# OSU-Nowlab/MPI4DL

Hardware: NVIDIA H100
Metric: images/sec (device-timed, max over ranks) AmoebaNet-D 8192^2 hot path (spatial-stage conv/pool fwd+bwd) (higher is better)
Workload: dtype bf16

## Files before the change

### mpi4dl_b200/build.py

```python
import os
import subprocess
import sys

HERE = os.path.dirname(os.path.abspath(__file__))
CSRC = os.path.join(HERE, "csrc")
LIB = os.path.join(HERE, "libspconv.so")
SOURCES = ["api.cu", "conv_direct.cu", "pool.cu", "halo.cu", "gemm_tc.cu", "conv_tap.cu", "wgrad_tap.cu", "bnrelu.cu",
           "halo_grad.cu", "gemm_tf32.cu", "conv_tap_tf32.cu", "conv_tap_s2_tf32.cu"]
NVCC_FLAGS = [
    "-O3", "-std=c++17", "-gencode", "arch=compute_90a,code=sm_90a", "-lineinfo",
    "-Xcompiler", "-fPIC", "--expt-relaxed-constexpr",
]


def _stale(target, deps):
    if not os.path.exists(target):
        return True
    t = os.path.getmtime(target)
    return any(os.path.getmtime(d) > t for d in deps)


def build_lib(force=False, verbose=False):
    nvcc = os.environ.get("NVCC", "/usr/local/cuda/bin/nvcc")
    hdrs = [os.path.join(CSRC, f) for f in os.listdir(CSRC) if f.endswith((".cuh", ".h"))]
    hdrs.append(os.path.join(HERE, "..", "include", "spconv.h"))
    objs = []
    procs = []
    for s in SOURCES:
        src = os.path.join(CSRC, s)
        obj = os.path.join(CSRC, s.replace(".cu", ".o"))
        objs.append(obj)
        if force or _stale(obj, [src] + hdrs):
            cmd = [nvcc] + NVCC_FLAGS + (["-Xptxas", "-v"] if verbose else []) + ["-c", src, "-o", obj]
            procs.append((s, subprocess.Popen(cmd, stdout=subprocess.PIPE, stderr=subprocess.STDOUT, text=True)))
    for s, p in procs:
        out, _ = p.communicate()
        if p.returncode != 0:
            sys.stderr.write(out)
            raise RuntimeError("nvcc failed on %s" % s)
        if verbose:
            sys.stderr.write(out)
    if force or procs or _stale(LIB, objs):
        cmd = [nvcc, "-shared", "-o", LIB] + objs + ["-gencode", "arch=compute_90a,code=sm_90a"]
        subprocess.check_call(cmd)
    return LIB


if __name__ == "__main__":
    print(build_lib(force="--force" in sys.argv, verbose="-v" in sys.argv))
```

### mpi4dl_b200/csrc/gemm_tc.cu

```cuda
#include <stdlib.h>

#include "common.cuh"
#include "tc_common.cuh"

namespace spc {

using namespace tc;

bool tap_v2_supported(int M, int Cin, int R, int S, int H, int W, int N, int stride);
int run_conv_tap_v2(const __nv_bfloat16* wp, int Mpad, int Cpad, const __nv_bfloat16* x, const __nv_bfloat16* bias,
                    __nv_bfloat16* y, int M, int Cin, int R, int S, int ph, int H, int W, int N, cudaStream_t st);

bool wgrad_tap_supported(int K, int C, int R, int S, int H, int W, int stride);
int run_wgrad_tap(const __nv_bfloat16* x, const __nv_bfloat16* dy, float* dw, int K, int C, int N, int H, int W, int R, int S,
                  cudaStream_t st);

namespace {

constexpr int TC_THREADS = 384;
constexpr int BK = 64;
constexpr int A_BLK_BYTES = 128 * BK * 2;
constexpr int B_BLK_BYTES = BK * 64 * 2;

typedef CUresult (*EncodeTiledFn)(CUtensorMap*, CUtensorMapDataType, cuuint32_t, void*, const cuuint64_t*,
                                  const cuuint64_t*, const cuuint32_t*, const cuuint32_t*, CUtensorMapInterleave,
                                  CUtensorMapSwizzle, CUtensorMapL2promotion, CUtensorMapFloatOOBfill);
EncodeTiledFn get_encode() {
  static EncodeTiledFn fn = nullptr;
  if (!fn) {
    void* p = nullptr;
    cudaDriverEntryPointQueryResult q;
    if (cudaGetDriverEntryPoint("cuTensorMapEncodeTiled", &p, cudaEnableDefault, &q) == cudaSuccess &&
        q == cudaDriverEntryPointSuccess)
      fn = reinterpret_cast<EncodeTiledFn>(p);
  }
  return fn;
}

int make_tmap_sw(CUtensorMap* m, const void* base, int rank, const uint64_t* dims, const uint64_t* strides_bytes,
                 const uint32_t* box, CUtensorMapSwizzle swz) {
  EncodeTiledFn enc = get_encode();
  if (!enc) {
    set_error("cuTensorMapEncodeTiled entry point not available");
    return SPC_ECUDA;
  }
  static thread_local bool ctx_bound = false;
  if (!ctx_bound) {
    if (cudaFree(nullptr) != cudaSuccess) {
      set_error("wgmma conv: no CUDA context on this thread");
      return SPC_ECUDA;
    }
    ctx_bound = true;
  }
  cuuint64_t gd[5], gs[5];
  cuuint32_t bx[5], es[5];
  for (int i = 0; i < rank; ++i) {
    gd[i] = dims[i];
    bx[i] = box[i];
    es[i] = 1;
    if (i > 0) gs[i - 1] = strides_bytes[i];
  }
  CUresult r = enc(m, CU_TENSOR_MAP_DATA_TYPE_BFLOAT16, (cuuint32_t)rank, const_cast<void*>(base), gd, gs, bx, es,
                   CU_TENSOR_MAP_INTERLEAVE_NONE, swz, CU_TENSOR_MAP_L2_PROMOTION_L2_256B,
                   CU_TENSOR_MAP_FLOAT_OOB_FILL_NONE);
  if (r != CUDA_SUCCESS) {
    set_error("cuTensorMapEncodeTiled failed (%d) rank=%d dims=[%llu,%llu,%llu] strides=[%llu,%llu]", (int)r, rank,
              (unsigned long long)dims[0], (unsigned long long)(rank > 1 ? dims[1] : 0),
              (unsigned long long)(rank > 2 ? dims[2] : 0), (unsigned long long)(rank > 1 ? strides_bytes[1] : 0),
              (unsigned long long)(rank > 2 ? strides_bytes[2] : 0));
    return SPC_ECUDA;
  }
  return SPC_OK;
}

int make_tmap(CUtensorMap* m, const void* base, int rank, const uint64_t* dims, const uint64_t* strides_bytes,
              const uint32_t* box) {
  return make_tmap_sw(m, base, rank, dims, strides_bytes, box, CU_TENSOR_MAP_SWIZZLE_128B);
}

__global__ void repack_weights_kernel(const __nv_bfloat16* __restrict__ w, __nv_bfloat16* __restrict__ wp, int M,
                                      int Cc, int Mpad, int Cpad, int taps, long long sm, long long sc, int flip) {
  const int total = taps * Mpad * Cpad;
  for (int i = blockIdx.x * blockDim.x + threadIdx.x; i < total; i += gridDim.x * blockDim.x) {
    const int c = i % Cpad;
    const int m = (i / Cpad) % Mpad;
    const int tap = i / (Cpad * Mpad);
    __nv_bfloat16 v = __float2bfloat16(0.f);
    if (m < M && c < Cc) v = w[(size_t)m * sm + (size_t)c * sc + (flip ? taps - 1 - tap : tap)];
    wp[i] = v;
  }
}

constexpr int BN = 128;
constexpr int OUT_BUF_BYTES = 128 * 128 * 2;
constexpr int MAX_STAGES = 8;

struct PwParams {
  int M;
// ... 187 lines not shown
struct EnvKnob { const char* name; const char* val; };
EnvKnob g_env_tab[32];
int g_env_n = 0;
inline const char* env_get(const char* name) {
  for (int i = 0; i < g_env_n; ++i)
    if (g_env_tab[i].name == name) return g_env_tab[i].val;
  const char* v = getenv(name);
  if (g_env_n < 32) { g_env_tab[g_env_n].name = name; g_env_tab[g_env_n].val = v; ++g_env_n; }
  return v;
}
inline int env_int(const char* name, int dflt) {
  const char* e = env_get(name);
  const int v = e ? atoi(e) : 0;
  return v > 0 ? v : dflt;
}
inline int sm_count() {
  static int sms = 0;
  if (!sms) {
    int dev = 0;
    cudaGetDevice(&dev);
    if (cudaDeviceGetAttribute(&sms, cudaDevAttrMultiProcessorCount, dev) != cudaSuccess || sms <= 0) sms = 132;
  }
  return sms;
}

constexpr int SMEM_LIMIT = 222 * 1024;
constexpr int SMEM_AUX = 1024  + 512 ;

template <int MB>
int launch_pw(const CUtensorMap& tw, const CUtensorMap& tx, const CUtensorMap& tx4, const CUtensorMap& ty, PwParams p,
              cudaStream_t st) {
  const int kchunks = (p.Cin + BK - 1) / BK;
  const int budget = SMEM_LIMIT - SMEM_AUX;
  const int wres_bytes = p.taps * kchunks * MB * A_BLK_BYTES;
  const int sms = sm_count();
  const int grid = p.num_tiles < sms ? p.num_tiles : sms;
  if (p.num_tiles < 16 * sms) p.tgroup = 1;
  p.wres = (wres_bytes <= 128 * 1024 && p.num_mg == 1) ? 1 : 0;
  const int stage_bytes = (p.wres ? 0 : MB * A_BLK_BYTES) + (BN / 64) * B_BLK_BYTES;
  const int rem = budget - (p.wres ? wres_bytes : 0);
  p.out_bufs = 2;
  p.stages = (rem - 2 * OUT_BUF_BYTES) / stage_bytes;
  if (p.stages < 3) { p.out_bufs = 1; p.stages = (rem - OUT_BUF_BYTES) / stage_bytes; }
  if (p.stages > MAX_STAGES) p.stages = MAX_STAGES;
  SPC_REQUIRE(p.stages >= 2, "wgmma conv: shared memory budget too small (MB=%d kchunks=%d)", MB, kchunks);
  const int smem = (p.wres ? wres_bytes : 0) + p.stages * stage_bytes + p.out_bufs * OUT_BUF_BYTES + SMEM_AUX;
  auto kern = pw_gemm_kernel<MB>;
  static bool attr_set = false;
  if (!attr_set) {
    SPC_CHECK_CUDA(cudaFuncSetAttribute(kern, cudaFuncAttributeMaxDynamicSharedMemorySize, SMEM_LIMIT));
    attr_set = true;
  }
  kern<<<grid, TC_THREADS, smem, st>>>(tw, tx, tx4, ty, p);
  count_launch();
  SPC_CHECK_CUDA(cudaGetLastError());
  return SPC_OK;
}

int make_act_tmap(CUtensorMap* m, const void* base, int P, int Cc, int N, int box_rows) {
  const uint64_t dims[3] = {(uint64_t)P, (uint64_t)Cc, (uint64_t)N};
  const uint64_t strides[3] = {0, (uint64_t)P * 2, (uint64_t)P * Cc * 2};
  const uint32_t box[3] = {64, (uint32_t)box_rows, 1};
  return make_tmap(m, base, 3, dims, strides, box);
}

int make_act_tmap5(CUtensorMap* m, const void* base, int P, int Cc, int N, int groups, int blocks) {
  const uint64_t dims[5] = {64, 8, (uint64_t)P / 64, (uint64_t)Cc / 8, (uint64_t)N};
  const uint64_t strides[5] = {0, (uint64_t)P * 2, 128, (uint64_t)P * 16, (uint64_t)P * Cc * 2};
  const uint32_t box[5] = {64, 8, (uint32_t)blocks, (uint32_t)groups, 1};
  return make_tmap(m, base, 5, dims, strides, box);
}

int launch_shift_copies(const void* x, void* xs, size_t planes, int H, int W, int S, int pw, int cs, cudaStream_t st);

struct TcConv {
  const __nv_bfloat16* w;
  long long sm, sc;
  int flip;
  int M, Cin;
  int R, S, ph, pw;
  int H, W, N;
  int stride;
  const __nv_bfloat16* prepacked;
};

int run_conv_tc(const TcConv& c, const __nv_bfloat16* x, const __nv_bfloat16* bias, __nv_bfloat16* y, void* ws,
                size_t ws_bytes, cudaStream_t st) {
  const int taps = c.R * c.S;
  const int cs = c.stride;
  const int Ho = c.H / cs, Wo = c.W / cs;
  const int Pin = c.H * c.W, P = Ho * Wo;
  const int Mpad = round_up(c.M, 128), Cpad = round_up(c.Cin, BK);
  const bool v2 = taps > 1 && !env_get("SPC_TAP_V1") && tap_v2_supported(c.M, c.Cin, c.R, c.S, c.H, c.W, c.N, cs);
  const bool copies = (c.S > 1 || cs > 1) && taps > 1 && !v2;
  const uintptr_t ws0 = reinterpret_cast<uintptr_t>(ws);
  const uintptr_t wp_addr = (ws0 + 1023) & ~(uintptr_t)1023;
  const size_t wp_bytes = c.prepacked ? 0 : (size_t)taps * Mpad * Cpad * 2;
  const uintptr_t xs_addr = (wp_addr + wp_bytes + 1023) & ~(uintptr_t)1023;
  const size_t xs_bytes = copies ? (size_t)c.S * c.N * c.Cin * c.H * Wo * 2 : 0;
  const size_t need = (xs_addr - ws0) + xs_bytes;
  SPC_REQUIRE((ws && ws_bytes >= need) || need <= 1024, "wgmma conv: workspace too small (%zu < %zu)", ws_bytes, need);
  const __nv_bfloat16* wp = c.prepacked;
  if (!c.prepacked) {
    __nv_bfloat16* wpm = reinterpret_cast<__nv_bfloat16*>(wp_addr);
    const int total = taps * Mpad * Cpad;
    int blocks = (total + 255) / 256;
    if (blocks > 1184) blocks = 1184;
    repack_weights_kernel<<<blocks, 256, 0, st>>>(c.w, wpm, c.M, c.Cin, Mpad, Cpad, taps, c.sm, c.sc, c.flip);
    count_launch();
    SPC_CHECK_CUDA(cudaGetLastError());
    wp = wpm;
  }
  if (v2)
    return run_conv_tap_v2(wp, Mpad, Cpad, x, bias, y, c.M, c.Cin, c.R, c.S, c.ph, c.H, c.W, c.N, st);
  const __nv_bfloat16* xsrc = x;
  if (copies) {
    void* xs = reinterpret_cast<void*>(xs_addr);
    int rc0 = launch_shift_copies(x, xs, (size_t)c.N * c.Cin, c.H, c.W, c.S, c.pw, cs, st);
    if (rc0) return rc0;
    xsrc = reinterpret_cast<const __nv_bfloat16*>(xs);
  }
  CUtensorMap tw, tx, tx4, ty;
  const char* box5_env = env_get("SPC_PW_BOX5");
  const int box5 = box5_env ? atoi(box5_env) : ((size_t)P * 2 >= ((size_t)4 << 20) ? 3 : 0);
  const int x5 = (taps == 1 && cs == 1 && (box5 & 1) && P % 64 == 0 && c.Cin % 8 == 0) ? 1 : 0;
  const int y5 = (taps == 1 && (box5 & 2) && P % 64 == 0 && c.M % 8 == 0) ? 1 : 0;
  {
    const uint64_t dims[2] = {(uint64_t)Cpad, (uint64_t)taps * Mpad};
    const uint64_t strides[2] = {0, (uint64_t)Cpad * 2};
    const uint32_t box[2] = {BK, 128};
    int rc = make_tmap(&tw, wp, 2, dims, strides, box);
    if (rc) return rc;
  }
  int rc;
  if (taps > 1) {
    const uint64_t dims[4] = {(uint64_t)Wo, (uint64_t)c.H, (uint64_t)c.Cin, (uint64_t)c.N * (copies ? c.S : 1)};
    const uint64_t strides[4] = {0, (uint64_t)Wo * 2, (uint64_t)c.H * Wo * 2, (uint64_t)c.H * Wo * c.Cin * 2};
    const uint32_t box[4] = {64, 1, BK, 1};
    rc = make_tmap(&tx4, xsrc, 4, dims, strides, box);
    if (rc) return rc;
    tx = tx4;
  } else {
    rc = x5 ? make_act_tmap5(&tx, x, Pin, c.Cin, c.N, BK / 8, BN / 64) : make_act_tmap(&tx, x, Pin, c.Cin, c.N, BK);
    if (rc) return rc;
    tx4 = tx;
  }
  rc = y5 ? make_act_tmap5(&ty, y, P, c.M, c.N, 16, 2) : make_act_tmap(&ty, y, P, c.M, c.N, 128);
  if (rc) return rc;
  PwParams p{};
  p.x5 = x5; p.y5 = y5;
  p.bias = bias; p.M = c.M; p.Cin = c.Cin; p.P = P; p.N = c.N;
  p.taps = taps; p.S = c.S; p.ph = c.ph; p.pw = c.pw; p.W = Wo; p.Mpad = Mpad;
  p.shiftN = copies ? c.N : 0;
  p.rowmul = cs;
  {
    const char* e = env_get("SPC_TILE_GROUP");
    p.tgroup = e ? atoi(e) : 1;
    if (p.tgroup < 1) p.tgroup = 1;
  }
  const int MBtot = Mpad / 128;
  const int mb = MBtot >= 2 ? 2 : 1;
  p.num_mg = (MBtot + mb - 1) / mb;
  p.tiles_per_image = (P + BN - 1) / BN;
  p.num_tiles = p.tiles_per_image * c.N * p.num_mg;
  return mb == 2 ? launch_pw<2>(tw, tx, tx4, ty, p, st) : launch_pw<1>(tw, tx, tx4, ty, p, st);
}

int run_pw(const __nv_bfloat16* w, int ld, int transpose, int M, int Cin, const __nv_bfloat16* x,
           const __nv_bfloat16* bias, __nv_bfloat16* y, int N, int P, void* ws, size_t ws_bytes, cudaStream_t st) {
  TcConv c{};
  c.w = w;
  c.sm = transpose ? 1 : ld; c.sc = transpose ? ld : 1; c.flip = 0;
  c.M = M; c.Cin = Cin; c.R = 1; c.S = 1; c.ph = 0; c.pw = 0; c.H = 1; c.W = P; c.N = N; c.stride = 1;
  return run_conv_tc(c, x, bias, y, ws, ws_bytes, st);
}

constexpr int WG_ACC = 256;

struct WgParams {
  float* dw;
  int K, C, P, N;
  int nblk;
  int n_blocks;
  int MG;
  int mgroups;
  int splits;
  int chunks_total;
  int chunks_per_image;
  int stages;
  int taps, S, ph;
  int TG, passes;
  int W, shiftN;
  int rowmul;
  int mrows;
  int split_major;
  int pb;
  int dy5, x5;
};

template <int NBLK, int NA>
__global__ void __launch_bounds__(TC_THREADS, 1)
pw_wgrad_kernel(const __grid_constant__ CUtensorMap tmap_dy, const __grid_constant__ CUtensorMap tmap_x,
                const __grid_constant__ CUtensorMap tmap_x4, const WgParams p) {
  static_assert(NA * NBLK <= WG_ACC, "accumulator registers");
  extern __shared__ uint8_t smem_raw[];
  uint8_t* smem = reinterpret_cast<uint8_t*>((reinterpret_cast<uintptr_t>(smem_raw) + 1023) & ~(uintptr_t)1023);
  const int MG = p.MG;
  const int b_bytes = NBLK * 128;
  const int b_slot = (b_bytes + 1023) & ~1023;
  const int stage_bytes = p.pb * (MG * A_BLK_BYTES + p.TG * b_slot);
  uint64_t* full = reinterpret_cast<uint64_t*>(smem + p.stages * stage_bytes);
  uint64_t* empty = full + MAX_STAGES;
  const int warp = threadIdx.x >> 5, lane = threadIdx.x & 31;

  if (threadIdx.x == 0) {
    for (int i = 0; i < p.stages; ++i) { mbar_init(&full[i], 1); mbar_init(&empty[i], 2); }
    fence_barrier_init();
  }
  __syncthreads();
  const int ngroups = p.mgroups * p.n_blocks * p.passes;
  const int num_items = ngroups * p.splits;
  const int per_split = (p.chunks_total + p.splits - 1) / p.splits;

#define WG_DECODE(it)                                                        \
  const int sp = p.split_major ? (it) / ngroups : (it) % p.splits;           \
  const int g_ = p.split_major ? (it) % ngroups : (it) / p.splits;           \
  const int pass = g_ % p.passes;                                            \
  const int nb = (g_ / p.passes) % p.n_blocks;                               \
  const int mgp = g_ / (p.passes * p.n_blocks);                              \
  const int tap0 = pass * p.TG;                                              \
  const int ntap = min(p.TG, p.taps - tap0);                                 \
  const int c_begin = sp * per_split, c_end = min(p.chunks_total, c_begin + per_split);

  if (warp == 0) {
    if (lane == 0) {
      tma_prefetch_desc(&tmap_dy);
      tma_prefetch_desc(&tmap_x);
      int s = 0, ph = 0;
      for (int it = blockIdx.x; it < num_items; it += gridDim.x) {
        WG_DECODE(it)
        for (int ch = c_begin; ch < c_end; ++ch) {
          const int n = ch / p.chunks_per_image, p0 = (ch % p.chunks_per_image) * (64 * p.pb);
          mbar_wait(&empty[s], ph ^ 1);
          uint8_t* st = smem + s * stage_bytes;
          mbar_arrive_expect_tx(&full[s], p.pb * (MG * p.mrows * 128 + ntap * b_bytes));
          if (p.pb == 2) {
            for (int i = 0; i < MG; ++i) {
              uint8_t* da = st + i * (2 * A_BLK_BYTES);
              const int r0 = (mgp * MG + i) * p.mrows;
              if (p.dy5) {
                tma_load_5d(da, &tmap_dy, &full[s], 0, 0, p0 >> 6, r0 >> 3, n);
              } else {
                tma_load_3d(da, &tmap_dy, &full[s], p0, r0, n);
// ... 549 lines not shown
    uintptr_t a = align1k(reinterpret_cast<uintptr_t>(ws));
    __nv_bfloat16* wq = reinterpret_cast<__nv_bfloat16*>(a);
    a = align1k(a + (size_t)4 * Mpad * Kpad * 2);
    __nv_bfloat16* tmp = reinterpret_cast<__nv_bfloat16*>(a);
    a = align1k(a + (size_t)4 * d->N * d->C * Ho * Wo * 2);
    {
      const int total = 4 * Mpad * Kpad;
      int blocks = (total + 255) / 256;
      if (blocks > 1184) blocks = 1184;
      repack_dgrad_s2_kernel<<<blocks, 256, 0, st>>>(reinterpret_cast<const __nv_bfloat16*>(w), wq, d->K, d->C, Mpad, Kpad);
      count_launch();
      SPC_CHECK_CUDA(cudaGetLastError());
    }
    TcConv c{};
    c.prepacked = wq;
    c.M = Mq; c.Cin = d->K; c.R = 2; c.S = 2; c.ph = 0; c.pw = 0; c.H = Ho; c.W = Wo; c.N = d->N; c.stride = 1;
    int rc = run_conv_tc(c, reinterpret_cast<const __nv_bfloat16*>(dy), nullptr, tmp, reinterpret_cast<void*>(a),
                         ws_bytes - (a - reinterpret_cast<uintptr_t>(ws)), st);
    if (rc) return rc;
    const size_t total = (size_t)d->N * d->C * 2 * Ho * (Wo / 8);
    size_t blocks = (total + 255) / 256;
    if (blocks > 132 * 32) blocks = 132 * 32;
    interleave_s2_kernel<<<(int)blocks, 256, 0, st>>>(tmp, reinterpret_cast<__nv_bfloat16*>(dx), d->N, d->C, Ho, Wo);
    count_launch();
    SPC_CHECK_CUDA(cudaGetLastError());
    return SPC_OK;
  }
  if (d->R * d->S > 1) {
    TcConv c{};
    c.w = reinterpret_cast<const __nv_bfloat16*>(w);
    c.sm = (long long)d->R * d->S; c.sc = (long long)d->C * d->R * d->S; c.flip = 1;
    c.M = d->C; c.Cin = d->K; c.R = d->R; c.S = d->S; c.ph = d->R - 1 - d->pad_h; c.pw = d->S - 1 - d->pad_w;
    c.H = d->H; c.W = d->W; c.N = d->N; c.stride = 1;
    return run_conv_tc(c, reinterpret_cast<const __nv_bfloat16*>(dy), nullptr, reinterpret_cast<__nv_bfloat16*>(dx), ws,
                       ws_bytes, st);
  }
  if (is_s2(d)) {
    void* gs = reinterpret_cast<void*>(align1k(reinterpret_cast<uintptr_t>(ws) + wbytes(d, 1)));
    int rc = run_pw(reinterpret_cast<const __nv_bfloat16*>(w), d->C, 1, d->C, d->K,
                    reinterpret_cast<const __nv_bfloat16*>(dy), nullptr, reinterpret_cast<__nv_bfloat16*>(gs), d->N,
                    (d->H / 2) * (d->W / 2), ws, wbytes(d, 1), st);
    if (rc) return rc;
    return launch_resample(true, gs, dx, (size_t)d->N * d->C, d->H, d->W, st);
  }
  return run_pw(reinterpret_cast<const __nv_bfloat16*>(w), d->C, 1, d->C, d->K,
                reinterpret_cast<const __nv_bfloat16*>(dy), nullptr, reinterpret_cast<__nv_bfloat16*>(dx), d->N,
                d->H * d->W, ws, ws_bytes, st);
}

int tc_conv_wgrad(const spc_conv_desc* d, const void* x, const void* dy, float* dw, int accumulate, void* ws,
                  size_t ws_bytes, cudaStream_t st) {
  (void)accumulate;
  const __nv_bfloat16* xb = reinterpret_cast<const __nv_bfloat16*>(x);
  const __nv_bfloat16* dyb = reinterpret_cast<const __nv_bfloat16*>(dy);
  if (d->R * d->S > 1) {
    const int cs = d->stride_h;
    if (!env_get("SPC_TAP_V1") && wgrad_tap_supported(d->K, d->C, d->R, d->S, d->H, d->W, cs))
      return run_wgrad_tap(xb, dyb, dw, d->K, d->C, d->N, d->H, d->W, d->R, d->S, st);
    const bool copies = d->S > 1 || cs > 1;
    if (copies) {
      SPC_REQUIRE(ws && ws_bytes >= tc_workspace_bytes(d, 2), "wgmma wgrad: workspace too small");
      void* xs = reinterpret_cast<void*>(align1k(reinterpret_cast<uintptr_t>(ws)));
      int rc = launch_shift_copies(x, xs, (size_t)d->N * d->C, d->H, d->W, d->S, d->pad_w, cs, st);
      if (rc) return rc;
      xb = reinterpret_cast<const __nv_bfloat16*>(xs);
    }
    return run_wgrad(xb, dyb, dw, d->K, d->C, d->N, d->H / cs, d->W / cs, d->H, d->R, d->S, d->pad_h, cs, copies, st);
  }
  if (is_s2(d)) {
    SPC_REQUIRE(ws && ws_bytes >= tc_workspace_bytes(d, 2), "wgmma wgrad: workspace too small");
    void* xs = reinterpret_cast<void*>(align1k(reinterpret_cast<uintptr_t>(ws)));
    int rc = launch_resample(false, x, xs, (size_t)d->N * d->C, d->H, d->W, st);
    if (rc) return rc;
    return run_wgrad(reinterpret_cast<const __nv_bfloat16*>(xs), dyb, dw, d->K, d->C, d->N, 1, (d->H / 2) * (d->W / 2), 1,
                     1, 1, 0, 1, false, st);
  }
  return run_wgrad(xb, dyb, dw, d->K, d->C, d->N, 1, d->H * d->W, 1, 1, 1, 0, 1, false, st);
}

size_t tc_pw_workspace_bytes(int M, int Cin) { return (size_t)round_up(M, 128) * round_up(Cin, BK) * 2 + 4096; }
int tc_pw_fwd(const void* w, int ld, int M, int Cin, const void* x, const void* bias, void* y, int P, void* ws, size_t ws_bytes,
              cudaStream_t st) {
  return run_pw(reinterpret_cast<const __nv_bfloat16*>(w), ld, 0, M, Cin, reinterpret_cast<const __nv_bfloat16*>(x),
                reinterpret_cast<const __nv_bfloat16*>(bias), reinterpret_cast<__nv_bfloat16*>(y), 1, P, ws, ws_bytes, st);
}
int tc_pw_wgrad(const void* x, const void* dy, float* dw, int K, int C, int P, cudaStream_t st) {
  return run_wgrad(reinterpret_cast<const __nv_bfloat16*>(x), reinterpret_cast<const __nv_bfloat16*>(dy), dw, K, C, 1, 1, P, 1, 1, 1,
                   0, 1, false, st);
}

int make_tmap_ex(CUtensorMap* m, const void* base, int rank, const uint64_t* dims, const uint64_t* strides_bytes,
                 const uint32_t* box, int swizzle128) {
  return make_tmap_sw(m, base, rank, dims, strides_bytes, box,
                      swizzle128 ? CU_TENSOR_MAP_SWIZZLE_128B : CU_TENSOR_MAP_SWIZZLE_NONE);
}
int tc_sm_count() { return sm_count(); }

}

extern "C" void spc_reload_env(void) { spc::g_env_n = 0; }
```

### mpi4dl_b200/csrc/wgmma.cuh

```cuda
#pragma once
#include <stdint.h>

namespace spc {
namespace tc {

template <int N, int TB> struct Wgmma;

template <int TB> struct Wgmma<16, TB> {
  static __device__ __forceinline__ void mma(float (&d)[8], uint64_t a, uint64_t b, uint32_t accumulate) {
    asm volatile(
        "{\n\t.reg .pred p;\n\t"
        "setp.ne.b32 p, %10, 0;\n\t"
        "wgmma.mma_async.sync.aligned.m64n16k16.f32.bf16.bf16 {%0, %1, %2, %3, %4, %5, %6, %7}, %8, %9, p, 1, 1, 0, %11;\n\t}"
        : "+f"(d[0]), "+f"(d[1]), "+f"(d[2]), "+f"(d[3]), "+f"(d[4]), "+f"(d[5]), "+f"(d[6]), "+f"(d[7])
        : "l"(a), "l"(b), "r"(accumulate), "n"(TB));
  }
};

template <int TB> struct Wgmma<32, TB> {
  static __device__ __forceinline__ void mma(float (&d)[16], uint64_t a, uint64_t b, uint32_t accumulate) {
    asm volatile(
        "{\n\t.reg .pred p;\n\t"
        "setp.ne.b32 p, %18, 0;\n\t"
        "wgmma.mma_async.sync.aligned.m64n32k16.f32.bf16.bf16 {%0, %1, %2, %3, %4, %5, %6, %7, %8, %9, %10, %11, %12, %13, %14, %15}, %16, %17, p, 1, 1, 0, %19;\n\t}"
        : "+f"(d[0]), "+f"(d[1]), "+f"(d[2]), "+f"(d[3]), "+f"(d[4]), "+f"(d[5]), "+f"(d[6]), "+f"(d[7]), "+f"(d[8]), "+f"(d[9]), "+f"(d[10]), "+f"(d[11]), "+f"(d[12]), "+f"(d[13]), "+f"(d[14]), "+f"(d[15])
        : "l"(a), "l"(b), "r"(accumulate), "n"(TB));
  }
};

template <int TB> struct Wgmma<48, TB> {
  static __device__ __forceinline__ void mma(float (&d)[24], uint64_t a, uint64_t b, uint32_t accumulate) {
    asm volatile(
        "{\n\t.reg .pred p;\n\t"
        "setp.ne.b32 p, %26, 0;\n\t"
        "wgmma.mma_async.sync.aligned.m64n48k16.f32.bf16.bf16 {%0, %1, %2, %3, %4, %5, %6, %7, %8, %9, %10, %11, %12, %13, %14, %15, %16, %17, %18, %19, %20, %21, %22, %23}, %24, %25, p, 1, 1, 0, %27;\n\t}"
        : "+f"(d[0]), "+f"(d[1]), "+f"(d[2]), "+f"(d[3]), "+f"(d[4]), "+f"(d[5]), "+f"(d[6]), "+f"(d[7]), "+f"(d[8]), "+f"(d[9]), "+f"(d[10]), "+f"(d[11]), "+f"(d[12]), "+f"(d[13]), "+f"(d[14]), "+f"(d[15]), "+f"(d[16]), "+f"(d[17]), "+f"(d[18]), "+f"(d[19]), "+f"(d[20]), "+f"(d[21]), "+f"(d[22]), "+f"(d[23])
        : "l"(a), "l"(b), "r"(accumulate), "n"(TB));
  }
};

template <int TB> struct Wgmma<64, TB> {
  static __device__ __forceinline__ void mma(float (&d)[32], uint64_t a, uint64_t b, uint32_t accumulate) {
    asm volatile(
        "{\n\t.reg .pred p;\n\t"
        "setp.ne.b32 p, %34, 0;\n\t"
        "wgmma.mma_async.sync.aligned.m64n64k16.f32.bf16.bf16 {%0, %1, %2, %3, %4, %5, %6, %7, %8, %9, %10, %11, %12, %13, %14, %15, %16, %17, %18, %19, %20, %21, %22, %23, %24, %25, %26, %27, %28, %29, %30, %31}, %32, %33, p, 1, 1, 0, %35;\n\t}"
        : "+f"(d[0]), "+f"(d[1]), "+f"(d[2]), "+f"(d[3]), "+f"(d[4]), "+f"(d[5]), "+f"(d[6]), "+f"(d[7]), "+f"(d[8]), "+f"(d[9]), "+f"(d[10]), "+f"(d[11]), "+f"(d[12]), "+f"(d[13]), "+f"(d[14]), "+f"(d[15]), "+f"(d[16]), "+f"(d[17]), "+f"(d[18]), "+f"(d[19]), "+f"(d[20]), "+f"(d[21]), "+f"(d[22]), "+f"(d[23]), "+f"(d[24]), "+f"(d[25]), "+f"(d[26]), "+f"(d[27]), "+f"(d[28]), "+f"(d[29]), "+f"(d[30]), "+f"(d[31])
        : "l"(a), "l"(b), "r"(accumulate), "n"(TB));
  }
};

template <int TB> struct Wgmma<80, TB> {
  static __device__ __forceinline__ void mma(float (&d)[40], uint64_t a, uint64_t b, uint32_t accumulate) {
    asm volatile(
        "{\n\t.reg .pred p;\n\t"
        "setp.ne.b32 p, %42, 0;\n\t"
        "wgmma.mma_async.sync.aligned.m64n80k16.f32.bf16.bf16 {%0, %1, %2, %3, %4, %5, %6, %7, %8, %9, %10, %11, %12, %13, %14, %15, %16, %17, %18, %19, %20, %21, %22, %23, %24, %25, %26, %27, %28, %29, %30, %31, %32, %33, %34, %35, %36, %37, %38, %39}, %40, %41, p, 1, 1, 0, %43;\n\t}"
        : "+f"(d[0]), "+f"(d[1]), "+f"(d[2]), "+f"(d[3]), "+f"(d[4]), "+f"(d[5]), "+f"(d[6]), "+f"(d[7]), "+f"(d[8]), "+f"(d[9]), "+f"(d[10]), "+f"(d[11]), "+f"(d[12]), "+f"(d[13]), "+f"(d[14]), "+f"(d[15]), "+f"(d[16]), "+f"(d[17]), "+f"(d[18]), "+f"(d[19]), "+f"(d[20]), "+f"(d[21]), "+f"(d[22]), "+f"(d[23]), "+f"(d[24]), "+f"(d[25]), "+f"(d[26]), "+f"(d[27]), "+f"(d[28]), "+f"(d[29]), "+f"(d[30]), "+f"(d[31]), "+f"(d[32]), "+f"(d[33]), "+f"(d[34]), "+f"(d[35]), "+f"(d[36]), "+f"(d[37]), "+f"(d[38]), "+f"(d[39])
        : "l"(a), "l"(b), "r"(accumulate), "n"(TB));
  }
};

template <int TB> struct Wgmma<96, TB> {
  static __device__ __forceinline__ void mma(float (&d)[48], uint64_t a, uint64_t b, uint32_t accumulate) {
    asm volatile(
        "{\n\t.reg .pred p;\n\t"
        "setp.ne.b32 p, %50, 0;\n\t"
        "wgmma.mma_async.sync.aligned.m64n96k16.f32.bf16.bf16 {%0, %1, %2, %3, %4, %5, %6, %7, %8, %9, %10, %11, %12, %13, %14, %15, %16, %17, %18, %19, %20, %21, %22, %23, %24, %25, %26, %27, %28, %29, %30, %31, %32, %33, %34, %35, %36, %37, %38, %39, %40, %41, %42, %43, %44, %45, %46, %47}, %48, %49, p, 1, 1, 0, %51;\n\t}"
        : "+f"(d[0]), "+f"(d[1]), "+f"(d[2]), "+f"(d[3]), "+f"(d[4]), "+f"(d[5]), "+f"(d[6]), "+f"(d[7]), "+f"(d[8]), "+f"(d[9]), "+f"(d[10]), "+f"(d[11]), "+f"(d[12]), "+f"(d[13]), "+f"(d[14]), "+f"(d[15]), "+f"(d[16]), "+f"(d[17]), "+f"(d[18]), "+f"(d[19]), "+f"(d[20]), "+f"(d[21]), "+f"(d[22]), "+f"(d[23]), "+f"(d[24]), "+f"(d[25]), "+f"(d[26]), "+f"(d[27]), "+f"(d[28]), "+f"(d[29]), "+f"(d[30]), "+f"(d[31]), "+f"(d[32]), "+f"(d[33]), "+f"(d[34]), "+f"(d[35]), "+f"(d[36]), "+f"(d[37]), "+f"(d[38]), "+f"(d[39]), "+f"(d[40]), "+f"(d[41]), "+f"(d[42]), "+f"(d[43]), "+f"(d[44]), "+f"(d[45]), "+f"(d[46]), "+f"(d[47])
        : "l"(a), "l"(b), "r"(accumulate), "n"(TB));
  }
};

template <int TB> struct Wgmma<112, TB> {
  static __device__ __forceinline__ void mma(float (&d)[56], uint64_t a, uint64_t b, uint32_t accumulate) {
    asm volatile(
        "{\n\t.reg .pred p;\n\t"
        "setp.ne.b32 p, %58, 0;\n\t"
        "wgmma.mma_async.sync.aligned.m64n112k16.f32.bf16.bf16 {%0, %1, %2, %3, %4, %5, %6, %7, %8, %9, %10, %11, %12, %13, %14, %15, %16, %17, %18, %19, %20, %21, %22, %23, %24, %25, %26, %27, %28, %29, %30, %31, %32, %33, %34, %35, %36, %37, %38, %39, %40, %41, %42, %43, %44, %45, %46, %47, %48, %49, %50, %51, %52, %53, %54, %55}, %56, %57, p, 1, 1, 0, %59;\n\t}"
        : "+f"(d[0]), "+f"(d[1]), "+f"(d[2]), "+f"(d[3]), "+f"(d[4]), "+f"(d[5]), "+f"(d[6]), "+f"(d[7]), "+f"(d[8]), "+f"(d[9]), "+f"(d[10]), "+f"(d[11]), "+f"(d[12]), "+f"(d[13]), "+f"(d[14]), "+f"(d[15]), "+f"(d[16]), "+f"(d[17]), "+f"(d[18]), "+f"(d[19]), "+f"(d[20]), "+f"(d[21]), "+f"(d[22]), "+f"(d[23]), "+f"(d[24]), "+f"(d[25]), "+f"(d[26]), "+f"(d[27]), "+f"(d[28]), "+f"(d[29]), "+f"(d[30]), "+f"(d[31]), "+f"(d[32]), "+f"(d[33]), "+f"(d[34]), "+f"(d[35]), "+f"(d[36]), "+f"(d[37]), "+f"(d[38]), "+f"(d[39]), "+f"(d[40]), "+f"(d[41]), "+f"(d[42]), "+f"(d[43]), "+f"(d[44]), "+f"(d[45]), "+f"(d[46]), "+f"(d[47]), "+f"(d[48]), "+f"(d[49]), "+f"(d[50]), "+f"(d[51]), "+f"(d[52]), "+f"(d[53]), "+f"(d[54]), "+f"(d[55])
        : "l"(a), "l"(b), "r"(accumulate), "n"(TB));
  }
};

template <int TB> struct Wgmma<128, TB> {
  static __device__ __forceinline__ void mma(float (&d)[64], uint64_t a, uint64_t b, uint32_t accumulate) {
    asm volatile(
        "{\n\t.reg .pred p;\n\t"
        "setp.ne.b32 p, %66, 0;\n\t"
        "wgmma.mma_async.sync.aligned.m64n128k16.f32.bf16.bf16 {%0, %1, %2, %3, %4, %5, %6, %7, %8, %9, %10, %11, %12, %13, %14, %15, %16, %17, %18, %19, %20, %21, %22, %23, %24, %25, %26, %27, %28, %29, %30, %31, %32, %33, %34, %35, %36, %37, %38, %39, %40, %41, %42, %43, %44, %45, %46, %47, %48, %49, %50, %51, %52, %53, %54, %55, %56, %57, %58, %59, %60, %61, %62, %63}, %64, %65, p, 1, 1, 0, %67;\n\t}"
        : "+f"(d[0]), "+f"(d[1]), "+f"(d[2]), "+f"(d[3]), "+f"(d[4]), "+f"(d[5]), "+f"(d[6]), "+f"(d[7]), "+f"(d[8]), "+f"(d[9]), "+f"(d[10]), "+f"(d[11]), "+f"(d[12]), "+f"(d[13]), "+f"(d[14]), "+f"(d[15]), "+f"(d[16]), "+f"(d[17]), "+f"(d[18]), "+f"(d[19]), "+f"(d[20]), "+f"(d[21]), "+f"(d[22]), "+f"(d[23]), "+f"(d[24]), "+f"(d[25]), "+f"(d[26]), "+f"(d[27]), "+f"(d[28]), "+f"(d[29]), "+f"(d[30]), "+f"(d[31]), "+f"(d[32]), "+f"(d[33]), "+f"(d[34]), "+f"(d[35]), "+f"(d[36]), "+f"(d[37]), "+f"(d[38]), "+f"(d[39]), "+f"(d[40]), "+f"(d[41]), "+f"(d[42]), "+f"(d[43]), "+f"(d[44]), "+f"(d[45]), "+f"(d[46]), "+f"(d[47]), "+f"(d[48]), "+f"(d[49]), "+f"(d[50]), "+f"(d[51]), "+f"(d[52]), "+f"(d[53]), "+f"(d[54]), "+f"(d[55]), "+f"(d[56]), "+f"(d[57]), "+f"(d[58]), "+f"(d[59]), "+f"(d[60]), "+f"(d[61]), "+f"(d[62]), "+f"(d[63])
        : "l"(a), "l"(b), "r"(accumulate), "n"(TB));
  }
};

}
}
```

Baseline: 3.227.

## Add pixel-major wgmma pointwise conv kernel with channel-sized N tiles

Adds a new warp-specialized wgmma GEMM for 1x1 convolutions where pixels form the M dimension (128 per tile) and output channels the N dimension, tiled at 56/104/208. It is used when the channel count pads poorly to 128-row tiles and there are enough tiles to fill the GPU. The intent is to cut wasted MMA work and padding for odd channel counts such as 52 or 208, and to keep weights resident in shared memory when they fit. The kernel uses transposed-A wgmma, stmatrix transpose for the epilogue, and TMA stores. It adds another code path and a layout, and it can run more slowly on shapes where the heuristic chooses poorly.

```diff
diff --git a/mpi4dl_b200/build.py b/mpi4dl_b200/build.py
--- a/mpi4dl_b200/build.py
+++ b/mpi4dl_b200/build.py
@@ -6,7 +6,8 @@
 CSRC = os.path.join(HERE, "csrc")
 LIB = os.path.join(HERE, "libspconv.so")
 SOURCES = ["api.cu", "conv_direct.cu", "pool.cu", "halo.cu", "gemm_tc.cu", "conv_tap.cu", "wgrad_tap.cu", "bnrelu.cu",
-           "halo_grad.cu", "gemm_tf32.cu", "conv_tap_tf32.cu", "conv_tap_s2_tf32.cu"]
+           "halo_grad.cu", "gemm_tf32.cu", "conv_tap_tf32.cu", "conv_tap_s2_tf32.cu",
+           "gemm_px.cu"]
 NVCC_FLAGS = [
     "-O3", "-std=c++17", "-gencode", "arch=compute_90a,code=sm_90a", "-lineinfo",
     "-Xcompiler", "-fPIC", "--expt-relaxed-constexpr",
diff --git a/mpi4dl_b200/csrc/gemm_px.cu b/mpi4dl_b200/csrc/gemm_px.cu
--- /dev/null
+++ b/mpi4dl_b200/csrc/gemm_px.cu
@@ -0,0 +1,232 @@
+#include "common.cuh"
+#include "tc_common.cuh"
+
+namespace spc {
+
+using namespace tc;
+
+namespace {
+
+constexpr int PX_THREADS = 384;
+constexpr int PX_BK = 64;
+constexpr int PX_BM = 128;
+constexpr int PX_X_BYTES = PX_BK * PX_BM * 2;
+constexpr int PX_MAX_STAGES = 8;
+constexpr int PX_SMEM_LIMIT = 222 * 1024;
+constexpr int PX_SMEM_AUX = 1024  + 512 ;
+
+struct PxParams {
+  int M;
+  int Cin;
+  int N, tiles_per_image;
+  int num_mg;
+  int num_tiles;
+  int stages;
+  int wres;
+  int out_bufs;
+  int x5, y5;
+  const __nv_bfloat16* bias;
+};
+
+__device__ __forceinline__ void stmatrix_x4_trans(uint32_t addr, uint32_t r0, uint32_t r1, uint32_t r2, uint32_t r3) {
+  asm volatile("stmatrix.sync.aligned.m8n8.x4.trans.shared.b16 [%0], {%1, %2, %3, %4};" ::"r"(addr), "r"(r0), "r"(r1),
+               "r"(r2), "r"(r3)
+               : "memory");
+}
+__device__ __forceinline__ void stmatrix_x2_trans(uint32_t addr, uint32_t r0, uint32_t r1) {
+  asm volatile("stmatrix.sync.aligned.m8n8.x2.trans.shared.b16 [%0], {%1, %2};" ::"r"(addr), "r"(r0), "r"(r1) : "memory");
+}
+
+template <int NT>
+__global__ void __launch_bounds__(PX_THREADS, 1)
+pw_px_gemm_kernel(const __grid_constant__ CUtensorMap tmap_w, const __grid_constant__ CUtensorMap tmap_x,
+                  const __grid_constant__ CUtensorMap tmap_y, const PxParams p) {
+  constexpr int W_BYTES = NT * 128;
+  constexpr int OUT_BYTES = NT * PX_BM * 2;
+  constexpr int NQ = NT / 8;
+  extern __shared__ uint8_t smem_raw[];
+  uint8_t* smem = reinterpret_cast<uint8_t*>((reinterpret_cast<uintptr_t>(smem_raw) + 1023) & ~(uintptr_t)1023);
+  const int kchunks = (p.Cin + PX_BK - 1) / PX_BK;
+  const int wres_bytes = p.wres ? kchunks * W_BYTES : 0;
+  const int stage_bytes = (p.wres ? 0 : W_BYTES) + PX_X_BYTES;
+  uint8_t* wres = smem;
+  uint8_t* stage0 = smem + wres_bytes;
+  uint8_t* outbuf = stage0 + p.stages * stage_bytes;
+  uint64_t* full = reinterpret_cast<uint64_t*>(outbuf + p.out_bufs * OUT_BYTES);
+  uint64_t* empty = full + PX_MAX_STAGES;
+  uint64_t* wfull = empty + PX_MAX_STAGES;
+  const int warp = threadIdx.x >> 5, lane = threadIdx.x & 31;
+  const bool x5 = p.x5, y5 = p.y5;
+
+  if (threadIdx.x == 0) {
+    for (int i = 0; i < p.stages; ++i) { mbar_init(&full[i], 1); mbar_init(&empty[i], 2); }
+    mbar_init(wfull, 1);
+    fence_barrier_init();
+  }
+  __syncthreads();
+
+  if (threadIdx.x < 128) {
+    setmaxnreg_dec<40>();
+    if (warp == 0 && lane == 0) {
+      tma_prefetch_desc(&tmap_w);
+      tma_prefetch_desc(&tmap_x);
+      if (p.wres) {
+        mbar_arrive_expect_tx(wfull, wres_bytes);
+        for (int kc = 0; kc < kchunks; ++kc) tma_load_2d(wres + kc * W_BYTES, &tmap_w, wfull, kc * PX_BK, 0);
+      }
+      int s = 0, ph = 0;
+      for (int t = blockIdx.x; t < p.num_tiles; t += gridDim.x) {
+        const int mg = t % p.num_mg, tt = t / p.num_mg;
+        const int n = tt / p.tiles_per_image, p0 = (tt % p.tiles_per_image) * PX_BM;
+        for (int kc = 0; kc < kchunks; ++kc) {
+          mbar_wait(&empty[s], ph ^ 1);
+          uint8_t* st = stage0 + s * stage_bytes;
+          mbar_arrive_expect_tx(&full[s], stage_bytes);
+          if (!p.wres) {
+            tma_load_2d(st, &tmap_w, &full[s], kc * PX_BK, mg * NT);
+            st += W_BYTES;
+          }
+          if (x5) {
+            tma_load_5d(st, &tmap_x, &full[s], 0, 0, p0 >> 6, kc * (PX_BK / 8), n);
+          } else {
+#pragma unroll
+            for (int j = 0; j < 2; ++j) tma_load_3d(st + j * (PX_X_BYTES / 2), &tmap_x, &full[s], p0 + 64 * j, kc * PX_BK, n);
+          }
+          if (++s == p.stages) { s = 0; ph ^= 1; }
+        }
+      }
+    }
+  } else {
+    setmaxnreg_inc<232>();
+    const int wg = (threadIdx.x >> 7) - 1;
+    const int w4 = (threadIdx.x >> 5) & 3;
+    const bool wg_lead = (threadIdx.x & 127) == 0;
+    const bool leader = threadIdx.x == 128;
+    const int mi = lane >> 3, cr = lane & 7;
+    const uint32_t blk = y5 ? 2048 : 1024;
+    const uint32_t lane_off = (y5 ? wg * 1024 : wg * W_BYTES) + (mi >> 1) * blk + cr * 128 +
+                              ((((16 * w4 + 8 * (mi & 1)) >> 3) ^ cr) << 4);
+    float acc[NT / 2];
+    if (p.wres) mbar_wait(wfull, 0);
+    int s = 0, ph = 0, ob = 0;
+    for (int t = blockIdx.x; t < p.num_tiles; t += gridDim.x) {
+      const int mg = t % p.num_mg, tt = t / p.num_mg;
+      const int n = tt / p.tiles_per_image, p0 = (tt % p.tiles_per_image) * PX_BM;
+      int prev = -1;
+      for (int kc = 0; kc < kchunks; ++kc) {
+        mbar_wait(&full[s], ph);
+        const uint32_t st = smem_u32(stage0 + s * stage_bytes);
+        const uint32_t sw = p.wres ? smem_u32(wres + kc * W_BYTES) : st;
+        const uint32_t sx = p.wres ? st : st + W_BYTES;
+        wgmma_fence();
+#pragma unroll
+        for (int ks = 0; ks < 4; ++ks) {
+          const uint64_t adesc = x5 ? gmma_desc(sx + wg * 1024 + ks * 4096, 1024, 2048)
+                                    : gmma_desc(sx + wg * (PX_X_BYTES / 2) + ks * 2048, PX_X_BYTES / 2, 1024);
+          const uint64_t bdesc = gmma_desc(sw + ks * 32, 16, 1024);
+          WgmmaTA<NT>::mma(acc, adesc, bdesc, (kc | ks) ? 1u : 0u);
+        }
+        wgmma_commit();
+        wgmma_wait<1>();
+        if (prev >= 0 && wg_lead) mbar_arrive(&empty[prev]);
+        prev = s;
+        if (++s == p.stages) { s = 0; ph ^= 1; }
+      }
+      wgmma_wait<0>();
+      reg_fence(acc);
+      if (prev >= 0 && wg_lead) mbar_arrive(&empty[prev]);
+      uint8_t* buf = outbuf + ob * OUT_BYTES;
+      if (leader) { if (p.out_bufs == 2) tma_store_wait_read<1>(); else tma_store_wait_read<0>(); }
+      named_bar_sync(1, 256);
+      {
+        const uint32_t base = smem_u32(buf) + lane_off;
+        const int k0 = mg * NT + 2 * (lane & 3);
+        float bv[NT / 4];
+#pragma unroll
+        for (int q = 0; q < NQ; ++q)
+#pragma unroll
+          for (int e = 0; e < 2; ++e) {
+            const int k = k0 + 8 * q + e;
+            bv[2 * q + e] = (p.bias && k < p.M) ? __bfloat162float(p.bias[k]) : 0.f;
+          }
+#pragma unroll
+        for (int q = 0; q + 1 < NQ; q += 2) {
+          stmatrix_x4_trans(base + q * blk,
+                            pack_bf16x2(acc[4 * q + 0] + bv[2 * q], acc[4 * q + 1] + bv[2 * q + 1]),
+                            pack_bf16x2(acc[4 * q + 2] + bv[2 * q], acc[4 * q + 3] + bv[2 * q + 1]),
+                            pack_bf16x2(acc[4 * q + 4] + bv[2 * q + 2], acc[4 * q + 5] + bv[2 * q + 3]),
+                            pack_bf16x2(acc[4 * q + 6] + bv[2 * q + 2], acc[4 * q + 7] + bv[2 * q + 3]));
+        }
+        if constexpr (NQ & 1) {
+          constexpr int q = NQ - 1;
+          stmatrix_x2_trans(base + q * blk,
+                            pack_bf16x2(acc[4 * q + 0] + bv[2 * q], acc[4 * q + 1] + bv[2 * q + 1]),
+                            pack_bf16x2(acc[4 * q + 2] + bv[2 * q], acc[4 * q + 3] + bv[2 * q + 1]));
+        }
+      }
+      fence_proxy_async();
+      named_bar_sync(1, 256);
+      if (leader) {
+        if (y5) {
+          tma_store_5d(&tmap_y, buf, 0, 0, p0 >> 6, (mg * NT) >> 3, n);
+        } else {
+#pragma unroll
+          for (int j = 0; j < 2; ++j) tma_store_3d(&tmap_y, buf + j * W_BYTES, p0 + 64 * j, mg * NT, n);
+        }
+        tma_store_commit();
+      }
+      if (p.out_bufs == 2) ob ^= 1;
+    }
+    if (leader) tma_store_wait_read<0>();
+  }
+}
+
+template <int NT>
+int launch_px(const CUtensorMap& tw, const CUtensorMap& tx, const CUtensorMap& ty, PxParams p, int sms,
+              cudaStream_t st) {
+  const int kchunks = (p.Cin + PX_BK - 1) / PX_BK;
+  const int budget = PX_SMEM_LIMIT - PX_SMEM_AUX;
+  const int wres_bytes = kchunks * NT * 128;
+  const int out_bytes = NT * PX_BM * 2;
+  int smem = 0;
+  for (int wres = (wres_bytes <= 128 * 1024 && p.num_mg == 1) ? 1 : 0; wres >= 0; --wres) {
+    const int stage_bytes = (wres ? 0 : NT * 128) + PX_X_BYTES;
+    const int rem = budget - (wres ? wres_bytes : 0);
+    p.wres = wres;
+    p.out_bufs = 2;
+    p.stages = (rem - 2 * out_bytes) / stage_bytes;
+    if (p.stages < 3) { p.out_bufs = 1; p.stages = (rem - out_bytes) / stage_bytes; }
+    if (p.stages > PX_MAX_STAGES) p.stages = PX_MAX_STAGES;
+    smem = (wres ? wres_bytes : 0) + p.stages * stage_bytes + p.out_bufs * out_bytes + PX_SMEM_AUX;
+    if (p.stages >= 2) break;
+  }
+  SPC_REQUIRE(p.stages >= 2, "wgmma px conv: shared memory budget too small (NT=%d kchunks=%d)", NT, kchunks);
+  auto kern = pw_px_gemm_kernel<NT>;
+  static bool attr_set = false;
+  if (!attr_set) {
+    SPC_CHECK_CUDA(cudaFuncSetAttribute(kern, cudaFuncAttributeMaxDynamicSharedMemorySize, PX_SMEM_LIMIT));
+    attr_set = true;
+  }
+  kern<<<p.num_tiles < sms ? p.num_tiles : sms, PX_THREADS, smem, st>>>(tw, tx, ty, p);
+  count_launch();
+  SPC_CHECK_CUDA(cudaGetLastError());
+  return SPC_OK;
+}
+
+}
+
+int run_pw_px(int NT, const CUtensorMap& tw, const CUtensorMap& tx, const CUtensorMap& ty, int M, int Cin, int N, int P,
+              int x5, int y5, const __nv_bfloat16* bias, int sms, cudaStream_t st) {
+  PxParams p{};
+  p.M = M; p.Cin = Cin; p.N = N; p.x5 = x5; p.y5 = y5; p.bias = bias;
+  p.num_mg = (M + NT - 1) / NT;
+  p.tiles_per_image = (P + PX_BM - 1) / PX_BM;
+  p.num_tiles = p.tiles_per_image * N * p.num_mg;
+  if (NT == 56) return launch_px<56>(tw, tx, ty, p, sms, st);
+  if (NT == 104) return launch_px<104>(tw, tx, ty, p, sms, st);
+  if (NT == 208) return launch_px<208>(tw, tx, ty, p, sms, st);
+  set_error("wgmma px conv: no kernel for %d output channels per tile", NT);
+  return SPC_EUNSUPPORTED;
+}
+
+}
diff --git a/mpi4dl_b200/csrc/gemm_tc.cu b/mpi4dl_b200/csrc/gemm_tc.cu
--- a/mpi4dl_b200/csrc/gemm_tc.cu
+++ b/mpi4dl_b200/csrc/gemm_tc.cu
@@ -14,6 +14,9 @@
 bool wgrad_tap_supported(int K, int C, int R, int S, int H, int W, int stride);
 int run_wgrad_tap(const __nv_bfloat16* x, const __nv_bfloat16* dy, float* dw, int K, int C, int N, int H, int W, int R, int S,
                   cudaStream_t st);
+
+int run_pw_px(int NT, const CUtensorMap& tw, const CUtensorMap& tx, const CUtensorMap& ty, int M, int Cin, int N, int P,
+              int x5, int y5, const __nv_bfloat16* bias, int sms, cudaStream_t st);
 
 namespace {
 
@@ -367,7 +370,16 @@
   int H, W, N;
   int stride;
   const __nv_bfloat16* prepacked;
+  int px;
 };
+
+int px_tile_channels(int M) {
+  const int nt = M <= 56 ? 56 : (M <= 104 ? 104 : 208);
+  const int pad = round_up(M, nt);
+  const int blocks = (M + 127) / 128;
+  const int old_rows = (blocks >= 2 ? round_up(blocks, 2) : 1) * 128;
+  return (pad < old_rows && 10 * M >= 9 * pad) ? nt : 0;
+}
 
 int run_conv_tc(const TcConv& c, const __nv_bfloat16* x, const __nv_bfloat16* bias, __nv_bfloat16* y, void* ws,
                 size_t ws_bytes, cudaStream_t st) {
@@ -375,7 +387,9 @@
   const int cs = c.stride;
   const int Ho = c.H / cs, Wo = c.W / cs;
   const int Pin = c.H * c.W, P = Ho * Wo;
-  const int Mpad = round_up(c.M, 128), Cpad = round_up(c.Cin, BK);
+  const int nt = (c.px && taps == 1) ? px_tile_channels(c.M) : 0;
+  const bool px = nt && (long long)c.N * ((P + BN - 1) / BN) >= 2ll * sm_count();
+  const int Mpad = round_up(c.M, px ? nt : 128), Cpad = round_up(c.Cin, BK);
   const bool v2 = taps > 1 && !env_get("SPC_TAP_V1") && tap_v2_supported(c.M, c.Cin, c.R, c.S, c.H, c.W, c.N, cs);
   const bool copies = (c.S > 1 || cs > 1) && taps > 1 && !v2;
   const uintptr_t ws0 = reinterpret_cast<uintptr_t>(ws);
@@ -413,11 +427,18 @@
   {
     const uint64_t dims[2] = {(uint64_t)Cpad, (uint64_t)taps * Mpad};
     const uint64_t strides[2] = {0, (uint64_t)Cpad * 2};
-    const uint32_t box[2] = {BK, 128};
+    const uint32_t box[2] = {BK, px ? (uint32_t)nt : 128u};
     int rc = make_tmap(&tw, wp, 2, dims, strides, box);
     if (rc) return rc;
   }
   int rc;
+  if (px) {
+    rc = x5 ? make_act_tmap5(&tx, x, Pin, c.Cin, c.N, BK / 8, BN / 64) : make_act_tmap(&tx, x, Pin, c.Cin, c.N, BK);
+    if (rc) return rc;
+    rc = y5 ? make_act_tmap5(&ty, y, P, c.M, c.N, nt / 8, 2) : make_act_tmap(&ty, y, P, c.M, c.N, nt);
+    if (rc) return rc;
+    return run_pw_px(nt, tw, tx, ty, c.M, c.Cin, c.N, P, x5, y5, bias, sm_count(), st);
+  }
   if (taps > 1) {
     const uint64_t dims[4] = {(uint64_t)Wo, (uint64_t)c.H, (uint64_t)c.Cin, (uint64_t)c.N * (copies ? c.S : 1)};
     const uint64_t strides[4] = {0, (uint64_t)Wo * 2, (uint64_t)c.H * Wo * 2, (uint64_t)c.H * Wo * c.Cin * 2};
@@ -452,8 +473,10 @@
 }
 
 int run_pw(const __nv_bfloat16* w, int ld, int transpose, int M, int Cin, const __nv_bfloat16* x,
-           const __nv_bfloat16* bias, __nv_bfloat16* y, int N, int P, void* ws, size_t ws_bytes, cudaStream_t st) {
+           const __nv_bfloat16* bias, __nv_bfloat16* y, int N, int P, void* ws, size_t ws_bytes, cudaStream_t st,
+           int px = 1) {
   TcConv c{};
+  c.px = px;
   c.w = w;
   c.sm = transpose ? 1 : ld; c.sc = transpose ? ld : 1; c.flip = 0;
   c.M = M; c.Cin = Cin; c.R = 1; c.S = 1; c.ph = 0; c.pw = 0; c.H = 1; c.W = P; c.N = N; c.stride = 1;
@@ -1169,7 +1192,8 @@
 int tc_pw_fwd(const void* w, int ld, int M, int Cin, const void* x, const void* bias, void* y, int P, void* ws, size_t ws_bytes,
               cudaStream_t st) {
   return run_pw(reinterpret_cast<const __nv_bfloat16*>(w), ld, 0, M, Cin, reinterpret_cast<const __nv_bfloat16*>(x),
-                reinterpret_cast<const __nv_bfloat16*>(bias), reinterpret_cast<__nv_bfloat16*>(y), 1, P, ws, ws_bytes, st);
+                reinterpret_cast<const __nv_bfloat16*>(bias), reinterpret_cast<__nv_bfloat16*>(y), 1, P, ws, ws_bytes, st,
+                0);
 }
 int tc_pw_wgrad(const void* x, const void* dy, float* dw, int K, int C, int P, cudaStream_t st) {
   return run_wgrad(reinterpret_cast<const __nv_bfloat16*>(x), reinterpret_cast<const __nv_bfloat16*>(dy), dw, K, C, 1, 1, P, 1, 1, 1,
diff --git a/mpi4dl_b200/csrc/wgmma.cuh b/mpi4dl_b200/csrc/wgmma.cuh
--- a/mpi4dl_b200/csrc/wgmma.cuh
+++ b/mpi4dl_b200/csrc/wgmma.cuh
@@ -94,5 +94,40 @@
   }
 };
 
+template <int N> struct WgmmaTA;
+
+template <> struct WgmmaTA<56> {
+  static __device__ __forceinline__ void mma(float (&d)[28], uint64_t a, uint64_t b, uint32_t accumulate) {
+    asm volatile(
+        "{\n\t.reg .pred p;\n\t"
+        "setp.ne.b32 p, %30, 0;\n\t"
+        "wgmma.mma_async.sync.aligned.m64n56k16.f32.bf16.bf16 {%0, %1, %2, %3, %4, %5, %6, %7, %8, %9, %10, %11, %12, %13, %14, %15, %16, %17, %18, %19, %20, %21, %22, %23, %24, %25, %26, %27}, %28, %29, p, 1, 1, 1, 0;\n\t}"
+        : "+f"(d[0]), "+f"(d[1]), "+f"(d[2]), "+f"(d[3]), "+f"(d[4]), "+f"(d[5]), "+f"(d[6]), "+f"(d[7]), "+f"(d[8]), "+f"(d[9]), "+f"(d[10]), "+f"(d[11]), "+f"(d[12]), "+f"(d[13]), "+f"(d[14]), "+f"(d[15]), "+f"(d[16]), "+f"(d[17]), "+f"(d[18]), "+f"(d[19]), "+f"(d[20]), "+f"(d[21]), "+f"(d[22]), "+f"(d[23]), "+f"(d[24]), "+f"(d[25]), "+f"(d[26]), "+f"(d[27])
+        : "l"(a), "l"(b), "r"(accumulate));
+  }
+};
+
+template <> struct WgmmaTA<104> {
+  static __device__ __forceinline__ void mma(float (&d)[52], uint64_t a, uint64_t b, uint32_t accumulate) {
+    asm volatile(
+        "{\n\t.reg .pred p;\n\t"
+        "setp.ne.b32 p, %54, 0;\n\t"
+        "wgmma.mma_async.sync.aligned.m64n104k16.f32.bf16.bf16 {%0, %1, %2, %3, %4, %5, %6, %7, %8, %9, %10, %11, %12, %13, %14, %15, %16, %17, %18, %19, %20, %21, %22, %23, %24, %25, %26, %27, %28, %29, %30, %31, %32, %33, %34, %35, %36, %37, %38, %39, %40, %41, %42, %43, %44, %45, %46, %47, %48, %49, %50, %51}, %52, %53, p, 1, 1, 1, 0;\n\t}"
+        : "+f"(d[0]), "+f"(d[1]), "+f"(d[2]), "+f"(d[3]), "+f"(d[4]), "+f"(d[5]), "+f"(d[6]), "+f"(d[7]), "+f"(d[8]), "+f"(d[9]), "+f"(d[10]), "+f"(d[11]), "+f"(d[12]), "+f"(d[13]), "+f"(d[14]), "+f"(d[15]), "+f"(d[16]), "+f"(d[17]), "+f"(d[18]), "+f"(d[19]), "+f"(d[20]), "+f"(d[21]), "+f"(d[22]), "+f"(d[23]), "+f"(d[24]), "+f"(d[25]), "+f"(d[26]), "+f"(d[27]), "+f"(d[28]), "+f"(d[29]), "+f"(d[30]), "+f"(d[31]), "+f"(d[32]), "+f"(d[33]), "+f"(d[34]), "+f"(d[35]), "+f"(d[36]), "+f"(d[37]), "+f"(d[38]), "+f"(d[39]), "+f"(d[40]), "+f"(d[41]), "+f"(d[42]), "+f"(d[43]), "+f"(d[44]), "+f"(d[45]), "+f"(d[46]), "+f"(d[47]), "+f"(d[48]), "+f"(d[49]), "+f"(d[50]), "+f"(d[51])
+        : "l"(a), "l"(b), "r"(accumulate));
+  }
+};
+
+template <> struct WgmmaTA<208> {
+  static __device__ __forceinline__ void mma(float (&d)[104], uint64_t a, uint64_t b, uint32_t accumulate) {
+    asm volatile(
+        "{\n\t.reg .pred p;\n\t"
+        "setp.ne.b32 p, %106, 0;\n\t"
+        "wgmma.mma_async.sync.aligned.m64n208k16.f32.bf16.bf16 {%0, %1, %2, %3, %4, %5, %6, %7, %8, %9, %10, %11, %12, %13, %14, %15, %16, %17, %18, %19, %20, %21, %22, %23, %24, %25, %26, %27, %28, %29, %30, %31, %32, %33, %34, %35, %36, %37, %38, %39, %40, %41, %42, %43, %44, %45, %46, %47, %48, %49, %50, %51, %52, %53, %54, %55, %56, %57, %58, %59, %60, %61, %62, %63, %64, %65, %66, %67, %68, %69, %70, %71, %72, %73, %74, %75, %76, %77, %78, %79, %80, %81, %82, %83, %84, %85, %86, %87, %88, %89, %90, %91, %92, %93, %94, %95, %96, %97, %98, %99, %100, %101, %102, %103}, %104, %105, p, 1, 1, 1, 0;\n\t}"
+        : "+f"(d[0]), "+f"(d[1]), "+f"(d[2]), "+f"(d[3]), "+f"(d[4]), "+f"(d[5]), "+f"(d[6]), "+f"(d[7]), "+f"(d[8]), "+f"(d[9]), "+f"(d[10]), "+f"(d[11]), "+f"(d[12]), "+f"(d[13]), "+f"(d[14]), "+f"(d[15]), "+f"(d[16]), "+f"(d[17]), "+f"(d[18]), "+f"(d[19]), "+f"(d[20]), "+f"(d[21]), "+f"(d[22]), "+f"(d[23]), "+f"(d[24]), "+f"(d[25]), "+f"(d[26]), "+f"(d[27]), "+f"(d[28]), "+f"(d[29]), "+f"(d[30]), "+f"(d[31]), "+f"(d[32]), "+f"(d[33]), "+f"(d[34]), "+f"(d[35]), "+f"(d[36]), "+f"(d[37]), "+f"(d[38]), "+f"(d[39]), "+f"(d[40]), "+f"(d[41]), "+f"(d[42]), "+f"(d[43]), "+f"(d[44]), "+f"(d[45]), "+f"(d[46]), "+f"(d[47]), "+f"(d[48]), "+f"(d[49]), "+f"(d[50]), "+f"(d[51]), "+f"(d[52]), "+f"(d[53]), "+f"(d[54]), "+f"(d[55]), "+f"(d[56]), "+f"(d[57]), "+f"(d[58]), "+f"(d[59]), "+f"(d[60]), "+f"(d[61]), "+f"(d[62]), "+f"(d[63]), "+f"(d[64]), "+f"(d[65]), "+f"(d[66]), "+f"(d[67]), "+f"(d[68]), "+f"(d[69]), "+f"(d[70]), "+f"(d[71]), "+f"(d[72]), "+f"(d[73]), "+f"(d[74]), "+f"(d[75]), "+f"(d[76]), "+f"(d[77]), "+f"(d[78]), "+f"(d[79]), "+f"(d[80]), "+f"(d[81]), "+f"(d[82]), "+f"(d[83]), "+f"(d[84]), "+f"(d[85]), "+f"(d[86]), "+f"(d[87]), "+f"(d[88]), "+f"(d[89]), "+f"(d[90]), "+f"(d[91]), "+f"(d[92]), "+f"(d[93]), "+f"(d[94]), "+f"(d[95]), "+f"(d[96]), "+f"(d[97]), "+f"(d[98]), "+f"(d[99]), "+f"(d[100]), "+f"(d[101]), "+f"(d[102]), "+f"(d[103])
+        : "l"(a), "l"(b), "r"(accumulate));
+  }
+};
+
 }
 }
```

After: 3.352 (median of 6 runs). 3.9% higher.
